# kssteven418/Q-ASR

Hardware: AMD Instinct MI355X
Metric: RTFx (audio-sec/wall-sec) QuartzNet15x5 int8 bs32 (higher is better)
Workload: dtype int8 (s8 x s8 -> i32 on MFMA; float64 fixed-point requant)

## Files before the change

### profiles/microbench/mel_cut.py

```python
import ctypes as C
import os
import subprocess
import sys
import tempfile

import numpy as np
import torch

ROOT = os.path.dirname(os.path.dirname(os.path.dirname(os.path.abspath(__file__))))
SRC = os.path.join(ROOT, 'q-asr_amd', 'csrc')
masks = [int(a) for a in sys.argv[1:]] or [0, 1, 2, 4, 8, 15, 31]
B, S, NM = 32, 80000, 64
dev = torch.device('cuda:0')
g = torch.Generator().manual_seed(0)
audio = (torch.randn(B, S, generator=g) * 0.1).to(dev)
lens = torch.full((B,), S, dtype=torch.int32, device=dev)
fb = torch.zeros(NM, 257)
edges = np.linspace(1, 256, NM + 2)
for m in range(NM):
    lo, c, hi = edges[m] ** 1.0, edges[m + 1], edges[m + 2]
    for k in range(257):
        if lo < k < hi:
            fb[m, k] = (k - lo) / (c - lo) if k <= c else (hi - k) / (hi - c)
fb = fb.to(dev)
win = torch.hann_window(320, periodic=False).to(dev)
tmp = tempfile.mkdtemp()
for mask in masks:
    so = os.path.join(tmp, f'fe{mask}.so')
    subprocess.check_call(['/opt/rocm/bin/hipcc', '--offload-arch=gfx950', '-O3', '-std=c++17', '-shared', '-fPIC',
                           f'-DMEL_CUT={mask}', '-I', os.path.join(ROOT, 'include'), '-o', so,
                           os.path.join(SRC, 'qasr_frontend.hip')])
    lib = C.CDLL(so)
    lib.qasr_frontend_frames.restype = C.c_int
    lib.qasr_frontend_workspace_bytes.restype = C.c_size_t
    T = lib.qasr_frontend_frames(S, 16)
    wsb = lib.qasr_frontend_workspace_bytes(B, S, NM)
    feats = torch.empty(B, NM, T, device=dev)
    fl = torch.empty(B, dtype=torch.int32, device=dev)
    ws = torch.empty(wsb, dtype=torch.uint8, device=dev)
    st = torch.cuda.current_stream()

    rc = lib.qasr_frontend_plan(C.c_void_p(st.cuda_stream), C.c_void_p(fb.data_ptr()), NM, C.c_void_p(ws.data_ptr()), C.c_size_t(wsb))
    assert rc == 0, rc

    def run():
        rc = lib.qasr_frontend_mel_planned(C.c_void_p(st.cuda_stream), C.c_void_p(audio.data_ptr()), C.c_void_p(lens.data_ptr()), B, S,
# ... 15 lines not shown
```

### q-asr_amd/csrc/qasr_decoder.hip

```cpp
#include "qasr_sep2_impl.h"

namespace qasr {

struct DecP {
  const int8_t* x;
  const int8_t* w;
  const int32_t* bias;
  const float* sb;
  const int32_t* lens;
  int32_t* lens_out;
  int32_t* acc_dbg;
  float* logits;
  float* logp;
  int32_t* tokens;
  float* frame_score;
  int cin, cin_pad, x_unsigned, B, T, Tp, ncls;
};

#define DEC_NT 512
#define DEC_TT 32

__global__ void __launch_bounds__(DEC_NT) k_dec(DecP p) {
  extern __shared__ __attribute__((aligned(16))) unsigned char smem[];
  const int tid = threadIdx.x, lane = tid & 63, h = lane >> 5;
  const int wave = __builtin_amdgcn_readfirstlane(tid >> 6);
  const int b = blockIdx.x, t0 = blockIdx.y * DEC_TT;
  lds_u8* const Xd = (lds_u8*)smem;
  int* const red = (int*)(smem + (size_t)p.cin_pad * 32);
  float* const lg = (float*)(red + 8 * 32 * 33);
  if (blockIdx.y == 0 && tid == 0 && p.lens_out) p.lens_out[b] = p.lens[b];
  const unsigned flip = p.x_unsigned ? 0x80808080u : 0u;
  for (int base = tid; base < 2 * p.cin_pad; base += 4 * DEC_NT) {
    v4i r[4];
#pragma unroll
    for (int u = 0; u < 4; ++u) {
      const int g = min(base + u * DEC_NT, 2 * p.cin_pad - 1), c = min(g >> 1, p.cin - 1), half = g & 1;
      r[u] = *(const v4i*)(p.x + ((size_t)b * p.cin + c) * p.Tp + t0 + 16 * half);
    }
#pragma unroll
    for (int u = 0; u < 4; ++u) {
      const int g = base + u * DEC_NT;
      if (g < 2 * p.cin_pad) {
        const int c = g >> 1, half = g & 1;
        v4i v = r[u];
        v[0] ^= flip, v[1] ^= flip, v[2] ^= flip, v[3] ^= flip;
        if (c >= p.cin) v = (v4i){0, 0, 0, 0};
        *(lds_v4i*)(Xd + c * 32 + 16 * half) = v;
      }
    }
  }
  __syncthreads();
  const int nks = p.cin_pad >> 5, per = nks >> 3;
  const lds_u8* const xd_lane = Xd + sep2_a_lane_off(lane);
  v16i acc;
#pragma unroll
  for (int r = 0; r < 16; ++r) acc[r] = 0;
  for (int i = 0; i < per; ++i) {
    const int ks = wave * per + i;
    const v4i a = sep2_a_frag(xd_lane, ks);
    const v4i wf = *w_frag(p.w, p.cin_pad, 0, ks);
    acc = __builtin_amdgcn_mfma_i32_32x32x32_i8(a, wf, acc, 0, 0, 0);
  }
#pragma unroll
  for (int r = 0; r < 16; ++r) red[(wave * 32 + mfma32_row(r, h)) * 33 + (lane & 31)] = acc[r];
  __syncthreads();
#pragma unroll
  for (int pass = 0; pass < 2; ++pass) {
    const int f = 16 * pass + (tid >> 5), c = tid & 31;
    int a = p.bias[c];
#pragma unroll
    for (int w = 0; w < 8; ++w) a += red[(w * 32 + f) * 33 + c];
    const int t = t0 + f;
    if (c < p.ncls && t < p.T) {
      if (p.acc_dbg) p.acc_dbg[((size_t)b * p.ncls + c) * p.Tp + t] = a;
      const float z = mul_f32_unfused((float)a, p.sb[c]);
      lg[f * 33 + c] = z;
      if (p.logits) p.logits[((size_t)b * p.T + t) * p.ncls + c] = z;
    }
  }
  __syncthreads();
  if (tid < DEC_TT && t0 + tid < p.T) {
    const float* x = lg + tid * 33;
    float m = x[0];
    int am = 0;
    for (int c = 1; c < p.ncls; ++c) {
      const float v = x[c];
      if (v > m) { m = v; am = c; }
    }
    float s = 0.f;
    for (int c = 0; c < p.ncls; ++c) s += expf(x[c] - m);
    const float ls = logf(s);
    const size_t row = (size_t)b * p.T + t0 + tid;
    if (p.logp)
      for (int c = 0; c < p.ncls; ++c) p.logp[row * p.ncls + c] = (x[c] - m) - ls;
    if (p.tokens) p.tokens[row] = am;
    if (p.frame_score) p.frame_score[row] = 0.0f - ls;
  }
}

bool decoder_fusable(const SepP& p) {
  return p.K == 0 && p.dense_k <= 1 && p.n_panes == 0 && (p.e.flags & QASR_F_LOGITS) && p.e.cout <= 32 && p.cin_pad % 256 == 0 &&
         p.cin_pad <= 2048 && p.e.Tp % DEC_TT == 0;
}

int launch_decoder(hipStream_t s, const SepP& q, float* logp, int32_t* tokens, int32_t* lens_out, bool keep_logits,
                   float* frame_score) {
  if (!decoder_fusable(q) || !q.x || !q.w || !q.bias || !q.e.sb || !q.e.lens || q.e.B < 1 || q.e.T > q.e.Tp) return QASR_ERR_ARG;
  DecP p{};
  p.x = q.x, p.w = q.w, p.bias = q.bias, p.sb = q.e.sb, p.lens = q.e.lens, p.lens_out = lens_out;
  p.acc_dbg = q.e.acc_dbg;
  p.logits = keep_logits ? q.e.logits : nullptr;
  p.logp = logp, p.tokens = tokens, p.frame_score = frame_score;
  p.cin = q.cin, p.cin_pad = q.cin_pad, p.x_unsigned = q.pw_unsigned;
  p.B = q.e.B, p.T = q.e.T, p.Tp = q.e.Tp, p.ncls = q.e.cout;
  const size_t smem = (size_t)p.cin_pad * 32 + sizeof(int) * 8 * 32 * 33 + sizeof(float) * 32 * 33;
  static int attr_dev = -1;
  int dev = 0;
  (void)hipGetDevice(&dev);
  if (attr_dev != dev) {
    (void)hipFuncSetAttribute((const void*)k_dec, hipFuncAttributeMaxDynamicSharedMemorySize, 160 * 1024);
    attr_dev = dev;
  }
  hipLaunchKernelGGL(k_dec, dim3(p.B, p.Tp / DEC_TT), dim3(DEC_NT), smem, s, p);
  return QASR_OK;
}

}
```

### q-asr_amd/csrc/qasr_engine.hip

```cpp
#include <algorithm>
#include <cstdarg>
#include <cstdio>
#include <cstdlib>
#include <cstring>
#include <string>
#include <type_traits>
#include <vector>

#include "qasr_internal.h"

#include <unordered_map>

using namespace qasr;

__global__ void __launch_bounds__(256) k_unpack6(const uint8_t* __restrict__ in, int8_t* __restrict__ out, size_t n_quads) {
  for (size_t q = blockIdx.x * (size_t)blockDim.x + threadIdx.x; q < n_quads; q += (size_t)gridDim.x * blockDim.x) {
    const unsigned w = in[3 * q] | ((unsigned)in[3 * q + 1] << 8) | ((unsigned)in[3 * q + 2] << 16);
    unsigned o = 0;
#pragma unroll
    for (int i = 0; i < 4; ++i) {
      const int c = (int)((w >> (6 * i)) & 0x3f);
      o |= (unsigned)(((c ^ 0x20) - 0x20) & 0xff) << (8 * i);
    }
    ((unsigned*)out)[q] = o;
// ... 56 lines not shown
  std::vector<std::vector<int32_t*>> acc_dbg;
  std::vector<hipEvent_t> ev;
  bool timed = false;
  bool fuse = true;
  std::vector<int> fused_dw;
  std::vector<char> skip;
  bool fuse_stem = true;
  bool stem = false;
  bool fuse_norm = true;
  double* norm_stats = nullptr;
  size_t norm_stats_bytes = 0;
  int norm_tiles = 0, norm_frames = 0;
  int fe_launches = 0;
  const int32_t* cur_lens = nullptr;
  bool fuse_dec = true;
  std::vector<char> rq_skip;
  std::vector<char> dec_skip;
  std::vector<char> dec_wide;
  void* decw_ws = nullptr;
  size_t decw_ws_bytes = 0;
  bool tile128 = true;
  int res_tile = 128;
  bool dense_tile128 = true;
  bool wide_tiles = false;
  int mask_skip = -1;
  int sep_gen = 2;
  bool forwarded = false;
  bool use_graph = false;
  hipGraphExec_t gexec = nullptr;
  const void* gkey[8] = {nullptr, nullptr, nullptr, nullptr, nullptr, nullptr, nullptr, nullptr};
// ... 95 lines not shown
  for (uint32_t d = 0; d < h.n_domains; ++d)
    if (e->domT[d] <= 0) return fail(QASR_ERR_ARG, "input of %d frames is too short for domain %u", T0, d);
  e->tens.resize(h.n_tensors);
  for (uint32_t i = 0; i < h.n_tensors; ++i) {
    TensorRT& t = e->tens[i];
    t.d = e->tdesc[i];
    t.T = e->domT[t.d.domain];
    t.Tp = rup(t.T, 64);
    t.bytes = (t.d.dtype == QASR_DT_F32) ? (size_t)B * t.T * t.d.channels * 4 : (size_t)B * t.d.channels * t.Tp * dt_size(t.d.dtype);
    t.bytes = (t.bytes + 255) / 256 * 256;
  }
  e->fused_dw.assign(h.n_ops, -1);
  e->skip.assign(h.n_ops, 0);
  e->dec_skip.assign(h.n_ops, 0);
  e->dec_wide.assign(h.n_ops, 0);
  e->rq_skip.assign(h.n_ops, 0);
  if (e->fuse)
    for (uint32_t oi = 0; oi + 1 < h.n_ops; ++oi) {
      const qasr_op_desc& d = e->ops[oi];
      const qasr_op_desc& q = e->ops[oi + 1];
      if (d.kind != QASR_OP_DW || q.kind != QASR_OP_PW) continue;
      const uint32_t same_pad = d.dilation > 1 ? (d.dilation * d.kernel) / 2 - 1 : d.kernel / 2;
      if (d.stride != 1 || d.padding != same_pad || !(d.kernel & 1) || !sep_supported((int)d.kernel, (int)d.dilation)) continue;
      if (d.outs[1].tensor >= 0 || d.outs[0].mode != 1 || q.in != d.outs[0].tensor) continue;
      if (e->tdesc[d.outs[0].tensor].last_use != (int)oi + 1 || (d.flags & QASR_F_EXACT_Z)) continue;
      e->fused_dw[oi + 1] = (int)oi;
      e->skip[oi] = 1;
    }
  e->B = B;
  e->T0 = T0;
// ... 161 lines not shown
  return QASR_OK;
}
int qasr_debug_timeline(void* dev_buf, size_t capacity_work_groups) {
  if (dev_buf && (capacity_work_groups < 1 || capacity_work_groups > (1u << 22))) return fail(QASR_ERR_ARG, "debug_timeline: capacity");
  qasr::g_prof = (long long*)dev_buf;
  qasr::g_prof_mode = dev_buf ? 1 : 0;
  qasr::g_prof_cap = dev_buf ? (int)capacity_work_groups : 0;
  return QASR_OK;
}

void qasr_engine_default_opts(qasr_engine_opts* o) {
  if (!o) return;
  memset(o, 0, sizeof *o);
  o->struct_size = (uint32_t)sizeof *o;
  o->fuse_dw = o->fuse_stem = o->fuse_decoder = o->res_tile128 = o->dense_tile128 = o->fuse_norm = o->mask_skip = -1;
}

#define QASR_SIDE_BY_SIDE_QUEUES 8
#define QASR_RES_TILE_FEW_CHAINS 64
static int res_tile_default() {
  long q = 4;
  if (const char* g = getenv("GPU_MAX_HW_QUEUES")) {
    char* end = nullptr;
    const long v = strtol(g, &end, 10);
    if (end != g && v >= 1) q = v;
  }
  return q >= QASR_SIDE_BY_SIDE_QUEUES ? 128 : QASR_RES_TILE_FEW_CHAINS;
}

int qasr_engine_create(const void* blob, size_t n, int device, int debug, qasr_engine** out) {
// ... 26 lines not shown
    char why[256];
    if (qasr_blob_check(blob, n, why, sizeof why) != QASR_OK) return fail(QASR_ERR_BLOB, "%s", why);
  }
  qasr_blob_header h;
  memcpy(&h, blob, sizeof h);
  HIPCHK(hipSetDevice(device));
  qasr_engine* e = new qasr_engine();
  e->device = device;
  e->debug = (debug & 1) != 0;
  e->timing = (debug & 3) != 0;
  auto tri = [](int32_t v, bool dflt) { return v < 0 ? dflt : v != 0; };
  e->fuse = tri(o.fuse_dw, true);
  e->fuse_stem = tri(o.fuse_stem, true);
  e->fuse_dec = tri(o.fuse_decoder, true);
  e->fuse_norm = tri(o.fuse_norm, true);
  e->wide_tiles = o.tile_frames >= 64;
  e->tile128 = o.tile_frames == 128;
  e->res_tile = o.res_tile128 < 0 ? res_tile_default() : (o.res_tile128 ? 128 : 64);
  e->dense_tile128 = tri(o.dense_tile128, true);
  e->sep_gen = o.sep_gen == 1 ? 1 : 2;
  e->mask_skip = o.mask_skip < 0 ? -1 : (o.mask_skip != 0);
  e->use_graph = o.graph > 0;
  if (getenv("QASR_NO_FUSE")) e->fuse = false;
  if (getenv("QASR_WIDE_TILES")) { e->wide_tiles = true; e->tile128 = true; }
  if (const char* g = getenv("QASR_TILE128")) e->tile128 = atoi(g) != 0;
  if (const char* g = getenv("QASR_RES_TILE128")) e->res_tile = atoi(g) != 0 ? 128 : 64;
  if (const char* g = getenv("QASR_RES_TILE")) {
    const int v = atoi(g);
    if (v == 32 || v == 64 || v == 128) e->res_tile = v;
  }
// ... 72 lines not shown
    if (bk.gexec) (void)hipGraphExecDestroy(bk.gexec);
  for (void* p : e->rs.owned) dev_free(e, p);
  free_plan(e);
  for (auto v : e->ev) (void)hipEventDestroy(v);
  dev_free(e, e->dblob);
  dev_free(e, e->dexp);
  delete e;
}

int qasr_engine_num_ops(const qasr_engine* e) { return e ? (int)e->h.n_ops : -1; }

int qasr_engine_num_launches(const qasr_engine* e) {
  if (!e || !e->B || !e->forwarded) return -1;
  int n = (e->stem ? 0 : 1) + e->fe_launches;
  for (uint32_t oi = 0; oi < e->h.n_ops; ++oi) {
    if (e->skip[oi] || e->dec_skip[oi] || e->rq_skip[oi] || (e->stem && oi >= 1 && oi <= 2)) continue;
    n += e->dec_wide[oi] ? 2 : 1;
  }
  return n + (e->ctc_on ? 1 : 0);
}

int qasr_engine_out_frames(const qasr_engine* e, int T) {
  if (!e) return -1;
  std::vector<int> dT(e->h.n_domains);
  dT[0] = T;
  for (uint32_t d = 1; d < e->h.n_domains; ++d) dT[d] = conv_out_len(dT[e->doms[d].parent], e->doms[d]);
  const qasr_op_desc& last = e->ops[e->h.n_ops - 1];
  return dT[e->tdesc[last.in].domain];
}

static void build_sep(qasr_engine* e, uint32_t oi, SepP& p) {
// ... 107 lines not shown
  QuantInP qi{};
  DwP dw{};
  SepP pw{};
  build_quant_in(e, 0, qi);
  build_dw(e, 1, dw);
  build_sep(e, 2, pw);
  int rc = launch_stem(s, qi, dw, pw, (const qasr_domain_desc*)(e->dblob + e->h.domains_off), (int)e->h.n_domains, e->cur_lens,
                       e->lens_all, e->norm_tiles ? e->norm_stats : nullptr, e->norm_tiles, e->norm_frames);
  return rc ? fail(rc, "k_stem launch") : QASR_OK;
}

static int launch_op(qasr_engine* e, hipStream_t s, uint32_t oi, float* logp, int32_t* tokens, int32_t* lens_out) {
  const qasr_op_desc& op = e->ops[oi];
  const int B = e->B;
  if (e->skip[oi]) return QASR_OK;
  if (e->stem && oi <= 2) return oi == 0 ? stem_launch(e, s) : QASR_OK;
  const TensorRT& tin = e->tens[op.in];
  switch (op.kind) {
    case QASR_OP_QUANT_IN: {
      QuantInP p{};
      build_quant_in(e, oi, p);
      launch_quant_in(s, p);
      break;
    }
    case QASR_OP_DW: {
      DwP p{};
      build_dw(e, oi, p);
      launch_dw(s, p);
      break;
    }
// ... 2 lines not shown
      build_sep(e, oi, p);
      if (e->fuse_dec && (op.flags & QASR_F_LOGITS) && oi + 1 < e->h.n_ops && e->ops[oi + 1].kind == QASR_OP_LOGSOFTMAX &&
          e->ops[oi + 1].in == op.outs[0].tensor && decoder_fusable(p)) {
        int rc = launch_decoder(s, p, logp, tokens, lens_out, e->debug, e->ctc_fs);
        if (rc) return fail(rc, "op %u: decoder launch", oi);
        e->dec_skip[oi + 1] = 1;
        break;
      }
      if (e->fuse_dec && (op.flags & QASR_F_LOGITS) && oi + 1 < e->h.n_ops && e->ops[oi + 1].kind == QASR_OP_LOGSOFTMAX &&
          e->ops[oi + 1].in == op.outs[0].tensor && decoder_wide_fusable(p)) {
        int rc = launch_decoder_wide(s, p, logp, tokens, lens_out, e->debug, e->decw_ws, e->decw_ws_bytes, e->ctc_fs);
        if (rc) return fail(rc, "op %u: wide decoder launch", oi);
        e->dec_skip[oi + 1] = 1;
        e->dec_wide[oi] = 1;
        break;
      }
      int rc = launch_sep(s, p);
      if (rc) return fail(rc, "op %u: no k_sep instantiation for K=%d dilation=%d (or bad launch shape)", oi, p.K, p.dilation);
      break;
    }
    case QASR_OP_DENSE: {
      if (op.flags & QASR_F_TAPMAJOR) {
        SepP p{};
        build_sep(e, oi, p);
        int rc = launch_sep(s, p);
        if (rc) return fail(rc, "op %u: dense conv has no k_sep launch shape", oi);
        break;
      }
      DenseP p{};
      p.x = (const int8_t*)tin.ptr;
// ... 1023 lines not shown
    HIPCHK(hipEventSynchronize(b));
    float ms = 0.f;
    HIPCHK(hipEventElapsedTime(&ms, a, b));
    ms_per_launch[oi] = ms / reps;
  }
  (void)hipEventDestroy(a);
  (void)hipEventDestroy(b);
  return QASR_OK;
}

int qasr_engine_op_label(qasr_engine* e, int op, char* buf, size_t cap) {
  if (!e || !buf || cap < 8 || op < 0 || op >= (int)e->h.n_ops) return fail(QASR_ERR_ARG, "op_label: bad argument");
  const qasr_op_desc& d = e->ops[op];
  const char* name = "?";
  if (e->skip[op]) name = "(fused into the next op)";
  else if (e->dec_skip[op]) name = "(fused into the previous op)";
  else if (e->rq_skip[op]) name = "(served by the previous k_requant launch)";
  else if (e->stem && op <= 2) name = op == 0 ? "k_stem" : "(fused into the first op)";
  else switch (d.kind) {
    case QASR_OP_QUANT_IN: name = "k_quant_in"; break;
    case QASR_OP_DW: name = "k_dw"; break;
    case QASR_OP_DENSE:
      if (d.flags & QASR_F_TAPMAJOR) {
        SepP p{};
        build_sep(e, (uint32_t)op, p);
        sep_kernel_label(p, buf, cap);
        return QASR_OK;
      }
      name = "k_dense";
      break;
    case QASR_OP_LOGSOFTMAX: name = "k_logsoftmax"; break;
// ... 271 lines not shown
```

### q-asr_amd/csrc/qasr_internal.h

```cpp
#pragma once
#include <hip/hip_runtime.h>
#include <stdint.h>

#include "../../include/qasr.h"

namespace qasr {

struct OutP {
  void* ptr;
  const double* mtab;
  double m;
  int lo, hi, mode;
  int pad_;
};

struct PaneP {
  const int8_t* x;
  const int8_t* w;
  const int32_t* bias;
  const double* m;
  const float* sb;
  int32_t* acc_dbg;
  int cin, cin_pad, x_unsigned, pad_;
};
// ... 97 lines not shown
size_t frontend_stats_bytes(int B, int S, int n_mels);
struct RaggedFront {
  int pitch, T_pad;
  const int32_t* shp;
};
int frontend_mel_stats(hipStream_t s, const float* audio, const int32_t* audio_lens, int B, int S, const float* fb,
                       const float* window, int n_mels, float preemph, int pad_to, float* feats, int32_t* feat_lens,
                       const void* workspace, size_t workspace_bytes, double* stats, int* n_tiles, int* n_frames,
                       const RaggedFront* rg = nullptr);
int frontend_mel_planned_ragged(hipStream_t s, const float* audio, const int32_t* audio_lens, int B, int S, const float* fb,
                                const float* window, int n_mels, float preemph, int pad_to, float* feats, int32_t* feat_lens,
                                const void* workspace, size_t workspace_bytes, const RaggedFront& rg);
bool decoder_fusable(const SepP& p);
int launch_decoder(hipStream_t s, const SepP& p, float* logp, int32_t* tokens, int32_t* lens_out, bool keep_logits,
                   float* frame_score = nullptr);
#define QASR_DECW_MAX_CLASSES 8192
bool decoder_wide_fusable(const SepP& p);
size_t decoder_wide_ws_bytes(int B, int Tp);
int launch_decoder_wide(hipStream_t s, const SepP& p, float* logp, int32_t* tokens, int32_t* lens_out, bool keep_logits,
                        void* ws, size_t ws_bytes, float* frame_score = nullptr);
int launch_ctc(hipStream_t s, const int32_t* tokens, const float* frame_score, const int32_t* lens, int B, int T, int blank,
               const qasr_ctc_out& out, const int32_t* t_act = nullptr);
int launch_topn(hipStream_t s, const qasr_ctc_topn_args& a);
size_t beam_workspace_bytes(int B, int T, int W);
int launch_beam(hipStream_t s, const qasr_ctc_beam_args& a);
int launch_beam_lm(hipStream_t s, const qasr_ctc_beam_lm_args& a);
int launch_beam_boost(hipStream_t s, const qasr_ctc_beam_boost_args& a);
size_t align_workspace_bytes(int P, int T, int max_labels);
int launch_align(hipStream_t s, const qasr_ctc_align_args& a);
size_t align_band_workspace_bytes(int P, int T, int band_states);
// ... 32 lines not shown
```

### q-asr_amd/csrc/qasr_sep2_impl.h

```cpp
#pragma once
#include <algorithm>
#include <cstdio>
#include <cstdlib>
#include <type_traits>

#include "qasr_device.h"

namespace qasr {

typedef int v2i __attribute__((ext_vector_type(2)));
typedef unsigned char __attribute__((address_space(3))) lds_u8;
typedef unsigned __attribute__((address_space(3))) lds_u32;
typedef v2i __attribute__((address_space(3))) lds_v2i;
typedef v4i __attribute__((address_space(3))) lds_v4i;

#define SEP2_NT 512
#ifndef SEP2_WPE
#define SEP2_WPE 2
#endif
#define SEP2_CH 128

template <int K, int TT>
struct Sep2Geo {
  static constexpr int PAD = K / 2;
// ... 154 lines not shown
      } else {
        if (r1) sep2_load_wg(&wf[4 * g], r1 + 256 * g);
      }
    }
    __builtin_amdgcn_sched_barrier(0);
  });
}

struct Sep2PassP {
  int bias, pbias;
  double Mo[QASR_MAX_OUTS];
  double Mm, Mp;
  float sbm, sbp;
};

template <int K, int NG, int NGP, int NP, bool DBG, int TT, int DIL = 1, bool SKIP = false>
__device__ __forceinline__ void sep2_body(const SepP& p, const int b, const int t0, const bool stamp_wg, const int wg_id) {
  using G = Sep2Geo<K, TT / DIL>;
  constexpr bool RES = NGP > 0;
  static_assert(DIL == 1 || (DIL == 2 && !RES && TT >= 64), "dilation 2: plain layers, 64- / 128-frame tiles");
  constexpr int MT = TT / 32;
  constexpr int NU = G::NU, S = G::S, NS = G::NS;
  constexpr int CIN_PAD = 128 * NG, PCIN_PAD = 128 * NGP;
  constexpr int RCH = 16 / DIL, GCH = SEP2_CH / DIL;
  constexpr int NCHUNK = (CIN_PAD + GCH - 1) / GCH;
  constexpr int NPGR = DIL == 1 ? G::NPG : (TT + 2 * DIL * G::HALO) / 16;
  constexpr int NPT = (RCH * NPGR + 63) / 64, NTG = RCH * G::KS / 16, NTT = (NTG + 63) / 64;
  static_assert(DIL == 1 || (8 * NPGR == G::WLEN && (RCH * G::KS) % 16 == 0), "dilation 2: window / tap granules");
  extern __shared__ __attribute__((aligned(16))) unsigned char smem[];
  const EpiP& e = p.e;
  int tid_ = threadIdx.x;
  asm volatile("" : "+v"(tid_));
  const int tid = tid_, lane = tid & 63, h = lane >> 5;
  const int wave = __builtin_amdgcn_readfirstlane(tid >> 6);
// ... 420 lines not shown
          }
        }
      };
      auto unit_values = [&](v16i* a, int ps, int mt0, auto v0c, auto v1c) __attribute__((always_inline)) {
        constexpr int v0 = decltype(v0c)::value, v1 = decltype(v1c)::value;
        sep2_for<v0, v1>([&](auto vc) {
          constexpr int v = decltype(vc)::value, mt = v / 16, r = v % 16;
          q4[r & 3] = rq_clamp(a[mt][r], pps[ps].Mo[0], olo, ohi);
          if constexpr ((r & 3) == 3) P[r >> 2] = pack4b(q4[0], q4[1], q4[2], q4[3]);
          if constexpr (r == 15) {
            const auto s02 = __builtin_amdgcn_permlane32_swap(P[0], P[2], false, false);
            const auto s13 = __builtin_amdgcn_permlane32_swap(P[1], P[3], false, false);
            v4i pk = {(int)s02[0], (int)s02[1], (int)s13[0], (int)s13[1]};
            if (t0 + 32 * (mt0 + mt + 1) > lim) pk = sep2_mask16(pk, lim - (t0 + 32 * (mt0 + mt) + 16 * h));
            *(v4i*)(optr + ((size_t)b * ecout + 256 * ps + co_l) * eTp + t0 + 32 * (mt0 + mt) + 16 * h) = pk;
          }
        });
      };
      auto u_ps = [](int u) constexpr { return u < NUN0 ? u / NH : NP - 1; };
      auto u_mh = [](int u) constexpr { return (SPLIT && u >= NUN0 - 1) ? 1 : MH; };
      auto u_mt0 = [](int u) constexpr { return u < NUN0 ? (u % NH) * MH : (NH - 1) * MH + 1; };
      sep2_for<0, NUN>([&](auto uc) {
        constexpr int u = decltype(uc)::value, ps = u_ps(u), mh = u_mh(u), mt0 = u_mt0(u);
        constexpr int AB = mh >= 2 ? 1 : 2, NSL = 4 * NG * mh;
        v16i* const cur = accs[u & 1];
#pragma unroll
        for (int mt = 0; mt < mh; ++mt)
#pragma unroll
          for (int r = 0; r < 16; ++r) cur[mt][r] = pps[ps].bias;
        const v4i* const wnext = (u < NUN0 && u % NH == NH - 1 && ps + 1 < NP) ? w_frag(p.w, CIN_PAD, 256 * (ps + 1) + co_l, 0) : nullptr;
        if constexpr (u > 0) unit_finish(accs[(u - 1) & 1], u_ps(u - 1), u_mt0(u - 1), std::integral_constant<int, u_mh(u - 1)>{});
        sep2_gemm_cb<mh, NG, 0, AB>(cur, wf, xd_lane + mt0 * (CIN_PAD * 32), CIN_PAD * 32, nullptr, wnext, [&](auto qc) {
          if constexpr (u > 0) {
            constexpr int NV = 16 * u_mh(u - 1), VPS = (NV + NSL - 1) / NSL;
            constexpr int q = decltype(qc)::value, v0 = q * VPS < NV ? q * VPS : NV, v1 = (q + 1) * VPS < NV ? (q + 1) * VPS : NV;
            unit_values(accs[(u - 1) & 1], u_ps(u - 1), u_mt0(u - 1), std::integral_constant<int, v0>{}, std::integral_constant<int, v1>{});
          }
        });
        STAMP2();
      });
      unit_finish(accs[(NUN - 1) & 1], NP - 1, u_mt0(NUN - 1), std::integral_constant<int, u_mh(NUN - 1)>{});
      unit_values(accs[(NUN - 1) & 1], NP - 1, u_mt0(NUN - 1), std::integral_constant<int, 0>{}, std::integral_constant<int, 16 * u_mh(NUN - 1)>{});
      STAMP2();
    }
  }
  if constexpr (!PIPED) {
#pragma unroll
  for (int ps = 0; ps < NP; ++ps) {
    const int cbase = 256 * ps;
    const int co = cbase + co_l, cor = co;
    constexpr bool co_ok = true;
    const bool more = ps + 1 < NP;
    const v4i* const wnext = more ? w_frag(p.w, CIN_PAD, co + 256, 0) : nullptr;
    const v4i* const wpane = RES ? w_frag(p.panes[0].w, PCIN_PAD, cor, 0) : nullptr;
    const Sep2PassP& pp = pps[ps];
    v16i acc[MT];
#pragma unroll
    for (int mt = 0; mt < MT; ++mt)
#pragma unroll
      for (int r = 0; r < 16; ++r) acc[mt][r] = pp.bias;
// ... 189 lines not shown
```

### q-asr_amd/qasr/engine.py

```python
import ctypes as C
import os

import numpy as np
import torch

HERE = os.path.dirname(os.path.abspath(__file__))
LIB_PATH = os.environ.get('QASR_LIB', os.path.join(HERE, 'libqasr_hip.so'))

SYMBOLS = ['qasr_blob_check', 'qasr_engine_create', 'qasr_engine_create_ex', 'qasr_engine_default_opts', 'qasr_engine_destroy', 'qasr_engine_forward', 'qasr_engine_forward_audio', 'qasr_engine_out_frames',
           'qasr_engine_num_ops', 'qasr_engine_num_launches', 'qasr_engine_read_acc', 'qasr_engine_read_tensor', 'qasr_engine_last_op_ms',
           'qasr_engine_time_ops', 'qasr_engine_run_op', 'qasr_engine_op_label',
           'qasr_frontend_mel', 'qasr_frontend_plan', 'qasr_frontend_mel_planned', 'qasr_frontend_frames',
           'qasr_frontend_workspace_bytes', 'qasr_pw_conv_acc',
           'qasr_dw_conv_acc', 'qasr_dense_conv_acc', 'qasr_requant', 'qasr_dyn_range', 'qasr_dyn_range_percentile', 'qasr_dyn_residue_codes', 'qasr_dyn_act_params', 'qasr_dyn_requant',
           'qasr_dyn_quant_in', 'qasr_dyn_conv_params', 'qasr_sep_layer', 'qasr_quantile2', 'qasr_quantile_workspace_bytes', 'qasr_debug_prof',
           'qasr_debug_timeline', 'qasr_ctc_collapse', 'qasr_engine_attach_ctc', 'qasr_ctc_topn', 'qasr_ctc_beam_workspace_bytes', 'qasr_ctc_beam',
           'qasr_lm_check', 'qasr_ctc_beam_lm', 'qasr_boost_check', 'qasr_ctc_beam_boost', 'qasr_ctc_align_workspace_bytes', 'qasr_ctc_align',
           'qasr_ctc_align_band_workspace_bytes', 'qasr_ctc_align_band',
           'qasr_engine_reserve', 'qasr_engine_forward_ragged', 'qasr_engine_forward_ragged_audio', 'qasr_engine_ragged_stats',
           'qasr_ragged_bucket_frames', 'qasr_ragged_envelope_frames',
           'qasr_resample_check', 'qasr_resample', 'qasr_resample_out_samples', 'qasr_longform_cut', 'qasr_longform_stitch',
           'qasr_stream_state_bytes', 'qasr_stream_push', 'qasr_stream_window', 'qasr_stream_emit',
           'qasr_last_error', 'qasr_version']

# ... 938 lines not shown
    for n in ('labels', 'start', 'nframes', 'score', 'n_new_labels', 'status', 'total_frames', 'utt_score'):
        setattr(a, n, getattr(out, n).data_ptr())
    if out.tail_labels is not None:
        assert out.tail_labels.dtype == torch.int32 and out.tail_labels.is_contiguous() and out.tail_labels.shape[0] == B, 'stream_emit: out'
        _i32dev(out.tail_n, B, 'stream_emit: out')
        a.Ptail, a.tail_labels, a.tail_n = out.tail_labels.shape[1], out.tail_labels.data_ptr(), out.tail_n.data_ptr()
    with torch.cuda.device(dev):
        _check(lib.qasr_stream_emit(_stream_ptr(stream), C.byref(a)), 'qasr_stream_emit')
    return out


class Engine:

    def __init__(self, blob: bytes, device=0, debug=False, timing=False, wide_tiles=False,
                 graph=False, tile=None, sep_gen=None, fuse_dw=None, fuse_stem=None, fuse_decoder=None, res_tile128=None,
                 dense_tile128=None, fuse_norm=None, legacy_create=False, mask_skip=None):
        lib = load_library()
        if not torch.cuda.is_available():
            raise QasrError('no GPU: the integer engine needs an MI355X (there is no CPU fallback)')
        self.lib = lib
        self.device = torch.device('cuda', device)
        self._blob = blob
        self._h = C.c_void_p()
        buf = (C.c_char * len(blob)).from_buffer_copy(blob)
        o = EngineOpts()
        lib.qasr_engine_default_opts(C.byref(o))
        assert o.struct_size == C.sizeof(EngineOpts), 'qasr_engine_opts: header and binding disagree'
        o.debug = int(bool(debug)) | (2 if timing else 0)
        o.tile_frames = int(tile) if tile else (128 if wide_tiles else 32)
        o.sep_gen = int(sep_gen or 0)
        for name, v in (('fuse_dw', fuse_dw), ('fuse_stem', fuse_stem), ('fuse_decoder', fuse_decoder),
                        ('res_tile128', res_tile128), ('dense_tile128', dense_tile128), ('fuse_norm', fuse_norm),
                        ('mask_skip', mask_skip)):
            if v is not None:
                setattr(o, name, int(bool(v)))
        o.graph = int(bool(graph))
        self.opts = o
        if legacy_create:
            bits = o.debug | (8 if o.tile_frames == 128 else 0) | (16 if graph else 0)
            _check(lib.qasr_engine_create(C.cast(buf, C.c_void_p), len(blob), device, bits, C.byref(self._h)), 'qasr_engine_create')
        else:
            _check(lib.qasr_engine_create_ex(C.cast(buf, C.c_void_p), len(blob), device, C.byref(o), C.byref(self._h)),
                   'qasr_engine_create_ex')
        self.debug = debug
        self.n_ops = lib.qasr_engine_num_ops(self._h)
        hdr = np.frombuffer(blob[:40], dtype=np.uint32)
        self.feat_in, self.n_classes = int(hdr[4]), int(hdr[5])
        self.B = self.T = None
        self._ctc = None
        self._ctc_auto = False
# ... 421 lines not shown
```

Measured before the change: 292,100.

## Fuse CTC decoder pointwise and log-softmax into the last encoder 1x1 layer

Adds a k_sep2_dec kernel in which the final 512->1024 pointwise encoder layer writes its int8 output tile into LDS through a tail hook. The same workgroup then runs the decoder 1x1 MFMA over that tile, the bias/scale reduction and the log-softmax/argmax. This removes the separate k_dec launch and the global re-read of the 1024-channel activation. In exchange the tile grows to a large LDS footprint (about 160 KB), which may lower occupancy of the encoder layer, and the extra decoder work lengthens each workgroup.

New measurement: 293,100, median of 4. About the same (+0.3%).

```diff
diff --git a/profiles/chain_ends.py b/profiles/chain_ends.py
--- /dev/null
+++ b/profiles/chain_ends.py
@@ -0,0 +1,125 @@
+#!/usr/bin/env python3
+import argparse
+import csv
+import glob
+import hashlib
+import json
+import os
+import shutil
+import statistics
+import subprocess
+import sys
+import tempfile
+
+ROOT = os.path.dirname(os.path.dirname(os.path.abspath(__file__)))
+ENDS = ('qasr::k_mel<', 'qasr::k_stem(', 'qasr::k_sep2<0, 4, 0, 4, false, 64, 1>', 'qasr::k_sep2_dec(', 'qasr::k_dec(',
+        'qasr::k_sep2<75, 4, 0, 2, false, 128, 1>')
+
+
+def lib_path(name):
+    return os.path.join(ROOT, 'q-asr_amd', 'qasr', f'libqasr_{name}.so')
+
+
+def bench_cmd(steps, warmup, extra=()):
+    return [sys.executable, os.path.join(ROOT, 'bench.py'), '--gpus', '1', '--steps', str(steps), '--warmup', str(warmup), *extra]
+
+
+def run_bench(build, queues, steps, warmup, extra=(), prefix=()):
+    env = dict(os.environ, QASR_LIB=lib_path(build), GPU_MAX_HW_QUEUES=str(queues))
+    p = subprocess.run([*prefix, *bench_cmd(steps, warmup, extra)], capture_output=True, text=True, env=env, timeout=400)
+    if p.returncode:
+        print(f'{build} (queues {queues}): FAILED rc={p.returncode}\n{p.stderr[-2000:]}', flush=True)
+        return None
+    d = json.loads([l for l in p.stdout.strip().splitlines() if l.startswith('{')][-1])
+    streams = [l.split('] ', 1)[1] for l in p.stderr.splitlines() if 'streams finished at' in l]
+    return dict(ms_per_step=d['ms_per_step'], rtfx=d['value'], streams=streams[0] if streams else None)
+
+
+def sha(path):
+    return hashlib.sha256(open(path, 'rb').read()).hexdigest()
+
+
+def main():
+    ap = argparse.ArgumentParser()
+    ap.add_argument('out')
+    ap.add_argument('--parent', default='parent')
+    ap.add_argument('--this', default='hip')
+    ap.add_argument('--rounds', type=int, default=3)
+    ap.add_argument('--steps', type=int, default=50)
+    ap.add_argument('--warmup', type=int, default=5)
+    ap.add_argument('--queues', type=int, nargs='+', default=[4, 8])
+    ap.add_argument('--stats', action='store_true')
+    a = ap.parse_args()
+    res = json.load(open(a.out)) if os.path.exists(a.out) else {}
+    builds = (a.parent, a.this)
+
+    def save():
+        with open(a.out, 'w') as fh:
+            json.dump(res, fh, indent=1)
+
+    if a.stats:
+        q = a.queues[0]
+        res['kernel_stats'] = dict(GPU_MAX_HW_QUEUES=q, steps=a.steps, warmup=a.warmup, rows={})
+        for build in builds:
+            tmp = tempfile.mkdtemp()
+            r = run_bench(build, q, a.steps, a.warmup, prefix=('rocprofv3', '--kernel-trace', '--stats', '--output-format', 'csv', '-d', tmp, '-o', 'p', '--'))
+            if r is None:
+                return 1
+            files = glob.glob(os.path.join(tmp, '**', '*kernel_stats.csv'), recursive=True)
+            rows = list(csv.reader(open(files[0])))
+            keep = [rows[0]] + [x for x in rows[1:] if 'qasr::' in x[0]]
+            with open(os.path.splitext(a.out)[0] + f'_kernel_stats_{build}.csv', 'w', newline='') as fh:
+                csv.writer(fh).writerows(keep)
+            ends = {}
+            for x in keep[1:]:
+                if any(k in x[0] for k in ENDS):
+                    name = x[0].replace('void ', '').split('(')[0]
+                    ends[name] = dict(calls=int(x[1]), mean_us=float(x[3]) / 1e3, min_us=float(x[5]) / 1e3, max_us=float(x[6]) / 1e3,
+                                      sigma_us=float(x[7]) / 1e3)
+            res['kernel_stats']['rows'][build] = dict(ms_per_step_under_rocprof=r['ms_per_step'], ends=ends)
+            shutil.rmtree(tmp, ignore_errors=True)
+            for k, v in ends.items():
+                print(f"{build:8s} {k:50s} {v['calls']:5d} calls  mean {v['mean_us']:7.2f}  max {v['max_us']:7.2f}  sigma {v['sigma_us']:6.2f} us", flush=True)
+            save()
+        return 0
+
+    runs = res.setdefault('runs', [])
+    for q in a.queues:
+        for r in range(a.rounds):
+            for build in builds:
+                rec = run_bench(build, q, a.steps, a.warmup)
+                if rec is None:
+                    return 1
+                rec.update(build=build, round=r, GPU_MAX_HW_QUEUES=q, steps=a.steps, warmup=a.warmup)
+                runs.append(rec)
+                print(f"{build:8s} queues {q:2d} round {r}  {rec['ms_per_step']:.4f} ms/step  {rec['streams']}", flush=True)
+                save()
+    summary = res.setdefault('summary', {})
+    for q in a.queues:
+        per = {b: sorted(x['ms_per_step'] for x in runs if x['build'] == b and x['GPU_MAX_HW_QUEUES'] == q) for b in builds}
+        summary[str(q)] = {b: dict(min=v[0], median=statistics.median(v), max=v[-1]) for b, v in per.items() if v}
+    if all(b in summary.get(str(a.queues[0]), {}) for b in builds):
+        s = summary[str(a.queues[0])]
+        summary['faster_than_every_parent_run'] = s[a.this]['max'] < s[a.parent]['min']
+    save()
+    hashes = res.setdefault('output_sha256', {})
+    for build in builds:
+        hashes[build] = {}
+        for extra in ((), ('--gather', 'logits')):
+            tmp = tempfile.mkdtemp()
+            if run_bench(build, a.queues[0], min(a.steps, 10), 2, extra=(*extra, '--dump-outputs', tmp)) is None:
+                return 1
+            for f in sorted(glob.glob(os.path.join(tmp, '*.npy'))):
+                name = os.path.basename(f)
+                if extra or name != 'log_probs.npy':
+                    h = sha(f)
+                    assert hashes[build].setdefault(name, h) == h, f'{build}: {name} differs between the two runs'
+            shutil.rmtree(tmp, ignore_errors=True)
+    res['outputs_identical'] = hashes[a.parent] == hashes[a.this] and len(hashes[a.this]) >= 3
+    save()
+    print(json.dumps(dict(summary=summary, outputs_identical=res['outputs_identical'], files=sorted(hashes[a.this])), indent=1), flush=True)
+    return 0 if res['outputs_identical'] else 2
+
+
+if __name__ == '__main__':
+    sys.exit(main())
diff --git a/profiles/microbench/mel_cut.py b/profiles/microbench/mel_cut.py
--- a/profiles/microbench/mel_cut.py
+++ b/profiles/microbench/mel_cut.py
@@ -27,9 +27,13 @@
 tmp = tempfile.mkdtemp()
 for mask in masks:
     so = os.path.join(tmp, f'fe{mask}.so')
-    subprocess.check_call(['/opt/rocm/bin/hipcc', '--offload-arch=gfx950', '-O3', '-std=c++17', '-shared', '-fPIC',
-                           f'-DMEL_CUT={mask}', '-I', os.path.join(ROOT, 'include'), '-o', so,
-                           os.path.join(SRC, 'qasr_frontend.hip')])
+    pre = os.path.join(os.environ.get('MEL_CUT_LIBS', tmp), f'fe{mask}.so')
+    if os.path.exists(pre):
+        so = pre
+    else:
+        subprocess.check_call(['/opt/rocm/bin/hipcc', '--offload-arch=gfx950', '-O3', '-std=c++17', '-shared', '-fPIC',
+                               f'-DMEL_CUT={mask}', '-I', os.path.join(ROOT, 'include'), '-o', so,
+                               os.path.join(SRC, 'qasr_frontend.hip')])
     lib = C.CDLL(so)
     lib.qasr_frontend_frames.restype = C.c_int
     lib.qasr_frontend_workspace_bytes.restype = C.c_size_t
diff --git a/q-asr_amd/csrc/qasr_decoder.hip b/q-asr_amd/csrc/qasr_decoder.hip
--- a/q-asr_amd/csrc/qasr_decoder.hip
+++ b/q-asr_amd/csrc/qasr_decoder.hip
@@ -20,9 +20,65 @@
 #define DEC_NT 512
 #define DEC_TT 32
 
+template <int NTL>
+__device__ __forceinline__ void dec_partial(const DecP& p, const lds_u8* Xd, int stride, int lane, int wave, v16i (&acc)[NTL]) {
+  const int nks = p.cin_pad >> 5, per = nks >> 3;
+  const lds_u8* const xd_lane = Xd + sep2_a_lane_off(lane);
+#pragma unroll
+  for (int n = 0; n < NTL; ++n)
+#pragma unroll
+    for (int r = 0; r < 16; ++r) acc[n][r] = 0;
+  for (int i = 0; i < per; ++i) {
+    const int ks = wave * per + i;
+    const v4i wf = *w_frag(p.w, p.cin_pad, 0, ks);
+#pragma unroll
+    for (int n = 0; n < NTL; ++n) {
+      const v4i a = sep2_a_frag(xd_lane + n * stride, ks);
+      acc[n] = __builtin_amdgcn_mfma_i32_32x32x32_i8(a, wf, acc[n], 0, 0, 0);
+    }
+  }
+}
+__device__ __forceinline__ void dec_put_partial(int* red, const v16i& acc, int lane, int wave) {
+  const int h = lane >> 5;
+#pragma unroll
+  for (int r = 0; r < 16; ++r) red[(wave * 32 + mfma32_row(r, h)) * 33 + (lane & 31)] = acc[r];
+}
+__device__ __forceinline__ void dec_reduce(const DecP& p, const int* red, float* lg, int b, int t0, int tid) {
+#pragma unroll
+  for (int pass = 0; pass < 2; ++pass) {
+    const int f = 16 * pass + (tid >> 5), c = tid & 31;
+    int a = p.bias[c];
+#pragma unroll
+    for (int w = 0; w < 8; ++w) a += red[(w * 32 + f) * 33 + c];
+    const int t = t0 + f;
+    if (c < p.ncls && t < p.T) {
+      if (p.acc_dbg) p.acc_dbg[((size_t)b * p.ncls + c) * p.Tp + t] = a;
+      const float z = mul_f32_unfused((float)a, p.sb[c]);
+      lg[f * 33 + c] = z;
+      if (p.logits) p.logits[((size_t)b * p.T + t) * p.ncls + c] = z;
+    }
+  }
+}
+__device__ __forceinline__ void dec_softmax(const DecP& p, const float* x, int b, int t) {
+  float m = x[0];
+  int am = 0;
+  for (int c = 1; c < p.ncls; ++c) {
+    const float v = x[c];
+    if (v > m) { m = v; am = c; }
+  }
+  float s = 0.f;
+  for (int c = 0; c < p.ncls; ++c) s += expf(x[c] - m);
+  const float ls = logf(s);
+  const size_t row = (size_t)b * p.T + t;
+  if (p.logp)
+    for (int c = 0; c < p.ncls; ++c) p.logp[row * p.ncls + c] = (x[c] - m) - ls;
+  if (p.tokens) p.tokens[row] = am;
+  if (p.frame_score) p.frame_score[row] = 0.0f - ls;
+}
+
 __global__ void __launch_bounds__(DEC_NT) k_dec(DecP p) {
   extern __shared__ __attribute__((aligned(16))) unsigned char smem[];
-  const int tid = threadIdx.x, lane = tid & 63, h = lane >> 5;
+  const int tid = threadIdx.x, lane = tid & 63;
   const int wave = __builtin_amdgcn_readfirstlane(tid >> 6);
   const int b = blockIdx.x, t0 = blockIdx.y * DEC_TT;
   lds_u8* const Xd = (lds_u8*)smem;
@@ -50,52 +106,60 @@
     }
   }
   __syncthreads();
-  const int nks = p.cin_pad >> 5, per = nks >> 3;
-  const lds_u8* const xd_lane = Xd + sep2_a_lane_off(lane);
-  v16i acc;
-#pragma unroll
-  for (int r = 0; r < 16; ++r) acc[r] = 0;
-  for (int i = 0; i < per; ++i) {
-    const int ks = wave * per + i;
-    const v4i a = sep2_a_frag(xd_lane, ks);
-    const v4i wf = *w_frag(p.w, p.cin_pad, 0, ks);
-    acc = __builtin_amdgcn_mfma_i32_32x32x32_i8(a, wf, acc, 0, 0, 0);
-  }
-#pragma unroll
-  for (int r = 0; r < 16; ++r) red[(wave * 32 + mfma32_row(r, h)) * 33 + (lane & 31)] = acc[r];
+  v16i acc[1];
+  dec_partial<1>(p, Xd, 0, lane, wave, acc);
+  dec_put_partial(red, acc[0], lane, wave);
   __syncthreads();
-#pragma unroll
-  for (int pass = 0; pass < 2; ++pass) {
-    const int f = 16 * pass + (tid >> 5), c = tid & 31;
-    int a = p.bias[c];
-#pragma unroll
-    for (int w = 0; w < 8; ++w) a += red[(w * 32 + f) * 33 + c];
-    const int t = t0 + f;
-    if (c < p.ncls && t < p.T) {
-      if (p.acc_dbg) p.acc_dbg[((size_t)b * p.ncls + c) * p.Tp + t] = a;
-      const float z = mul_f32_unfused((float)a, p.sb[c]);
-      lg[f * 33 + c] = z;
-      if (p.logits) p.logits[((size_t)b * p.T + t) * p.ncls + c] = z;
-    }
-  }
+  dec_reduce(p, red, lg, b, t0, tid);
   __syncthreads();
-  if (tid < DEC_TT && t0 + tid < p.T) {
-    const float* x = lg + tid * 33;
-    float m = x[0];
-    int am = 0;
-    for (int c = 1; c < p.ncls; ++c) {
-      const float v = x[c];
-      if (v > m) { m = v; am = c; }
-    }
-    float s = 0.f;
-    for (int c = 0; c < p.ncls; ++c) s += expf(x[c] - m);
-    const float ls = logf(s);
-    const size_t row = (size_t)b * p.T + t0 + tid;
-    if (p.logp)
-      for (int c = 0; c < p.ncls; ++c) p.logp[row * p.ncls + c] = (x[c] - m) - ls;
-    if (p.tokens) p.tokens[row] = am;
-    if (p.frame_score) p.frame_score[row] = 0.0f - ls;
-  }
+  if (tid < DEC_TT && t0 + tid < p.T) dec_softmax(p, lg + tid * 33, b, t0 + tid);
+}
+
+#define TAIL_TT 64
+#define TAIL_CIN 512
+#define TAIL_CMID 1024
+#define TAIL_IMG (TAIL_TT * TAIL_CIN)
+#define TAIL_RED (TAIL_IMG + TAIL_TT * TAIL_CMID)
+#define TAIL_LG (TAIL_RED + 4 * 8 * 32 * 33)
+#define TAIL_SMEM (TAIL_LG + 4 * TAIL_TT * 33)
+static_assert(TAIL_SMEM <= 160 * 1024, "k_sep2_dec: LDS budget");
+
+struct Sep2DecTail {
+  static constexpr bool on = true;
+  const DecP& d;
+  unsigned char* smem;
+  lds_u8* lds;
+  unsigned flip;
+  __device__ __forceinline__ void put(int mt, int ch, int h, v4i pk) const {
+    pk[0] ^= flip, pk[1] ^= flip, pk[2] ^= flip, pk[3] ^= flip;
+    *(lds_v4i*)(lds + TAIL_IMG + mt * (32 * TAIL_CMID) + ch * 32 + 16 * h) = pk;
+  }
+  __device__ __forceinline__ void run(int b, int t0, int tid) const {
+    const int lane = tid & 63, wave = __builtin_amdgcn_readfirstlane(tid >> 6);
+    int* const red = (int*)(smem + TAIL_RED);
+    float* const lg = (float*)(smem + TAIL_LG);
+    if (t0 == 0 && tid == 0 && d.lens_out) d.lens_out[b] = d.lens[b];
+    __syncthreads();
+    v16i acc[2];
+    dec_partial<2>(d, lds + TAIL_IMG, 32 * TAIL_CMID, lane, wave, acc);
+#pragma unroll
+    for (int n = 0; n < 2; ++n) {
+      if (n) __syncthreads();
+      dec_put_partial(red, acc[n], lane, wave);
+      __syncthreads();
+      dec_reduce(d, red, lg + n * (DEC_TT * 33), b, t0 + DEC_TT * n, tid);
+    }
+    __syncthreads();
+    if (tid < TAIL_TT && t0 + tid < d.T) dec_softmax(d, lg + tid * 33, b, t0 + tid);
+  }
+};
+
+__global__ void __launch_bounds__(SEP2_NT, SEP2_WPE) k_sep2_dec(SepP p, DecP d) {
+  extern __shared__ __attribute__((aligned(16))) unsigned char smem[];
+  static_assert(SEP2_NT == DEC_NT, "the decoder's thread layout");
+  const Sep2DecTail tail{d, smem, (lds_u8*)smem, d.x_unsigned ? 0x80808080u : 0u};
+  sep2_body<0, TAIL_CIN / 128, 0, TAIL_CMID / 256, false, TAIL_TT, 1, false, Sep2DecTail>(
+      p, blockIdx.x, blockIdx.y * TAIL_TT, blockIdx.x == 0 && blockIdx.y == 1, blockIdx.y * gridDim.x + blockIdx.x, tail);
 }
 
 bool decoder_fusable(const SepP& p) {
@@ -103,16 +167,20 @@
          p.cin_pad <= 2048 && p.e.Tp % DEC_TT == 0;
 }
 
-int launch_decoder(hipStream_t s, const SepP& q, float* logp, int32_t* tokens, int32_t* lens_out, bool keep_logits,
-                   float* frame_score) {
-  if (!decoder_fusable(q) || !q.x || !q.w || !q.bias || !q.e.sb || !q.e.lens || q.e.B < 1 || q.e.T > q.e.Tp) return QASR_ERR_ARG;
-  DecP p{};
+static void dec_params(DecP& p, const SepP& q, float* logp, int32_t* tokens, int32_t* lens_out, bool keep_logits, float* frame_score) {
   p.x = q.x, p.w = q.w, p.bias = q.bias, p.sb = q.e.sb, p.lens = q.e.lens, p.lens_out = lens_out;
   p.acc_dbg = q.e.acc_dbg;
   p.logits = keep_logits ? q.e.logits : nullptr;
   p.logp = logp, p.tokens = tokens, p.frame_score = frame_score;
   p.cin = q.cin, p.cin_pad = q.cin_pad, p.x_unsigned = q.pw_unsigned;
   p.B = q.e.B, p.T = q.e.T, p.Tp = q.e.Tp, p.ncls = q.e.cout;
+}
+
+int launch_decoder(hipStream_t s, const SepP& q, float* logp, int32_t* tokens, int32_t* lens_out, bool keep_logits,
+                   float* frame_score) {
+  if (!decoder_fusable(q) || !q.x || !q.w || !q.bias || !q.e.sb || !q.e.lens || q.e.B < 1 || q.e.T > q.e.Tp) return QASR_ERR_ARG;
+  DecP p{};
+  dec_params(p, q, logp, tokens, lens_out, keep_logits, frame_score);
   const size_t smem = (size_t)p.cin_pad * 32 + sizeof(int) * 8 * 32 * 33 + sizeof(float) * 32 * 33;
   static int attr_dev = -1;
   int dev = 0;
@@ -125,4 +193,33 @@
   return QASR_OK;
 }
 
-}
+bool decoder_tail_fusable(const SepP& enc, const SepP& dec) {
+  const EpiP& e = enc.e;
+  if (!decoder_fusable(dec) || dec.e.acc_dbg || dec.cin != TAIL_CMID || dec.cin_pad != TAIL_CMID) return false;
+  if (enc.gen != 2 || !sep2_shape_ok(enc) || enc.K != 0 || enc.cin_pad != TAIL_CIN || e.cout != TAIL_CMID || enc.tile < 64) return false;
+  if (enc.mask_skip || e.acc_dbg || enc.dw_acc_dbg || g_prof) return false;
+  return e.n_outs == 1 && e.outs[0].ptr == (const void*)dec.x && e.B == dec.e.B && e.T == dec.e.T && e.Tp == dec.e.Tp && e.Tp % TAIL_TT == 0;
+}
+
+int launch_decoder_tail(hipStream_t s, const SepP& enc, const SepP& dec, float* logp, int32_t* tokens, int32_t* lens_out, float* frame_score) {
+  if (!decoder_tail_fusable(enc, dec) || !enc.x || !enc.w || !dec.x || !dec.w || !dec.bias || !dec.e.sb || !dec.e.lens || dec.e.B < 1 ||
+      dec.e.T > dec.e.Tp)
+    return QASR_ERR_ARG;
+  DecP d{};
+  dec_params(d, dec, logp, tokens, lens_out, false, frame_score);
+  SepP q = enc;
+  q.prof = nullptr;
+  q.prof_mode = 0;
+  q.prof_cap = 0;
+  static int attr_dev = -1;
+  int dev = 0;
+  (void)hipGetDevice(&dev);
+  if (attr_dev != dev) {
+    (void)hipFuncSetAttribute((const void*)k_sep2_dec, hipFuncAttributeMaxDynamicSharedMemorySize, 160 * 1024);
+    attr_dev = dev;
+  }
+  hipLaunchKernelGGL(k_sep2_dec, dim3(q.e.B, q.e.Tp / TAIL_TT, 1), dim3(SEP2_NT), (size_t)TAIL_SMEM, s, q, d);
+  return QASR_OK;
+}
+
+}
diff --git a/q-asr_amd/csrc/qasr_engine.hip b/q-asr_amd/csrc/qasr_engine.hip
--- a/q-asr_amd/csrc/qasr_engine.hip
+++ b/q-asr_amd/csrc/qasr_engine.hip
@@ -94,6 +94,8 @@
   int fe_launches = 0;
   const int32_t* cur_lens = nullptr;
   bool fuse_dec = true;
+  bool fuse_tail = true;
+  std::vector<char> tail_skip;
   std::vector<char> rq_skip;
   std::vector<char> dec_skip;
   std::vector<char> dec_wide;
@@ -219,6 +221,7 @@
   e->skip.assign(h.n_ops, 0);
   e->dec_skip.assign(h.n_ops, 0);
   e->dec_wide.assign(h.n_ops, 0);
+  e->tail_skip.assign(h.n_ops, 0);
   e->rq_skip.assign(h.n_ops, 0);
   if (e->fuse)
     for (uint32_t oi = 0; oi + 1 < h.n_ops; ++oi) {
@@ -410,6 +413,7 @@
   memset(o, 0, sizeof *o);
   o->struct_size = (uint32_t)sizeof *o;
   o->fuse_dw = o->fuse_stem = o->fuse_decoder = o->res_tile128 = o->dense_tile128 = o->fuse_norm = o->mask_skip = -1;
+  o->reserved[0] = -1;
 }
 
 #define QASR_SIDE_BY_SIDE_QUEUES 8
@@ -466,6 +470,7 @@
   e->fuse_stem = tri(o.fuse_stem, true);
   e->fuse_dec = tri(o.fuse_decoder, true);
   e->fuse_norm = tri(o.fuse_norm, true);
+  e->fuse_tail = tri(o.reserved[0], true);
   e->wide_tiles = o.tile_frames >= 64;
   e->tile128 = o.tile_frames == 128;
   e->res_tile = o.res_tile128 < 0 ? res_tile_default() : (o.res_tile128 ? 128 : 64);
@@ -568,7 +573,7 @@
   if (!e || !e->B || !e->forwarded) return -1;
   int n = (e->stem ? 0 : 1) + e->fe_launches;
   for (uint32_t oi = 0; oi < e->h.n_ops; ++oi) {
-    if (e->skip[oi] || e->dec_skip[oi] || e->rq_skip[oi] || (e->stem && oi >= 1 && oi <= 2)) continue;
+    if (e->skip[oi] || e->dec_skip[oi] || e->tail_skip[oi] || e->rq_skip[oi] || (e->stem && oi >= 1 && oi <= 2)) continue;
     n += e->dec_wide[oi] ? 2 : 1;
   }
   return n + (e->ctc_on ? 1 : 0);
@@ -706,6 +711,7 @@
   const qasr_op_desc& op = e->ops[oi];
   const int B = e->B;
   if (e->skip[oi]) return QASR_OK;
+  if (e->tail_skip[oi]) return QASR_OK;
   if (e->stem && oi <= 2) return oi == 0 ? stem_launch(e, s) : QASR_OK;
   const TensorRT& tin = e->tens[op.in];
   switch (op.kind) {
@@ -738,6 +744,21 @@
         e->dec_skip[oi + 1] = 1;
         e->dec_wide[oi] = 1;
         break;
+      }
+      if (e->fuse_dec && e->fuse_tail && !e->debug && !e->timing && !e->rs.on && oi + 2 < e->h.n_ops) {
+        const qasr_op_desc &d1 = e->ops[oi + 1], &d2 = e->ops[oi + 2];
+        if (d1.kind == QASR_OP_PW && (d1.flags & QASR_F_LOGITS) && d1.in == op.outs[0].tensor && d2.kind == QASR_OP_LOGSOFTMAX &&
+            d2.in == d1.outs[0].tensor) {
+          SepP pd{};
+          build_sep(e, oi + 1, pd);
+          if (decoder_tail_fusable(p, pd)) {
+            int rc = launch_decoder_tail(s, p, pd, logp, tokens, lens_out, e->ctc_fs);
+            if (rc) return fail(rc, "op %u: decoder launch inside the previous layer's", oi + 1);
+            e->tail_skip[oi + 1] = 1;
+            e->dec_skip[oi + 2] = 1;
+            break;
+          }
+        }
       }
       int rc = launch_sep(s, p);
       if (rc) return fail(rc, "op %u: no k_sep instantiation for K=%d dilation=%d (or bad launch shape)", oi, p.K, p.dilation);
@@ -1791,7 +1812,7 @@
   const qasr_op_desc& d = e->ops[op];
   const char* name = "?";
   if (e->skip[op]) name = "(fused into the next op)";
-  else if (e->dec_skip[op]) name = "(fused into the previous op)";
+  else if (e->dec_skip[op] || e->tail_skip[op]) name = "(fused into the previous op)";
   else if (e->rq_skip[op]) name = "(served by the previous k_requant launch)";
   else if (e->stem && op <= 2) name = op == 0 ? "k_stem" : "(fused into the first op)";
   else switch (d.kind) {
diff --git a/q-asr_amd/csrc/qasr_internal.h b/q-asr_amd/csrc/qasr_internal.h
--- a/q-asr_amd/csrc/qasr_internal.h
+++ b/q-asr_amd/csrc/qasr_internal.h
@@ -135,6 +135,9 @@
 bool decoder_fusable(const SepP& p);
 int launch_decoder(hipStream_t s, const SepP& p, float* logp, int32_t* tokens, int32_t* lens_out, bool keep_logits,
                    float* frame_score = nullptr);
+bool decoder_tail_fusable(const SepP& enc, const SepP& dec);
+int launch_decoder_tail(hipStream_t s, const SepP& enc, const SepP& dec, float* logp, int32_t* tokens, int32_t* lens_out,
+                        float* frame_score = nullptr);
 #define QASR_DECW_MAX_CLASSES 8192
 bool decoder_wide_fusable(const SepP& p);
 size_t decoder_wide_ws_bytes(int B, int Tp);
diff --git a/q-asr_amd/csrc/qasr_sep2_impl.h b/q-asr_amd/csrc/qasr_sep2_impl.h
--- a/q-asr_amd/csrc/qasr_sep2_impl.h
+++ b/q-asr_amd/csrc/qasr_sep2_impl.h
@@ -192,10 +192,15 @@
   float sbm, sbp;
 };
 
-template <int K, int NG, int NGP, int NP, bool DBG, int TT, int DIL = 1, bool SKIP = false>
-__device__ __forceinline__ void sep2_body(const SepP& p, const int b, const int t0, const bool stamp_wg, const int wg_id) {
+struct Sep2NoTail {
+  static constexpr bool on = false;
+};
+template <int K, int NG, int NGP, int NP, bool DBG, int TT, int DIL = 1, bool SKIP = false, class TAIL = Sep2NoTail>
+__device__ __forceinline__ void sep2_body(const SepP& p, const int b, const int t0, const bool stamp_wg, const int wg_id,
+                                          const TAIL tail = TAIL{}) {
   using G = Sep2Geo<K, TT / DIL>;
   constexpr bool RES = NGP > 0;
+  static_assert(!TAIL::on || (K == 0 && !RES && !DBG && !SKIP && TT == 64), "the tail hook: the bare 1x1 form on 64-frame tiles");
   static_assert(DIL == 1 || (DIL == 2 && !RES && TT >= 64), "dilation 2: plain layers, 64- / 128-frame tiles");
   constexpr int MT = TT / 32;
   constexpr int NU = G::NU, S = G::S, NS = G::NS;
@@ -646,6 +651,7 @@
             v4i pk = {(int)s02[0], (int)s02[1], (int)s13[0], (int)s13[1]};
             if (t0 + 32 * (mt0 + mt + 1) > lim) pk = sep2_mask16(pk, lim - (t0 + 32 * (mt0 + mt) + 16 * h));
             *(v4i*)(optr + ((size_t)b * ecout + 256 * ps + co_l) * eTp + t0 + 32 * (mt0 + mt) + 16 * h) = pk;
+            if constexpr (TAIL::on) tail.put(mt0 + mt, 256 * ps + co_l, h, pk);
           }
         });
       };
@@ -676,6 +682,8 @@
       STAMP2();
     }
   }
+  static_assert(!TAIL::on || PIPED, "the tail hook sits in the pipelined epilogue");
+  if constexpr (TAIL::on) tail.run(b, t0, tid);
   if constexpr (!PIPED) {
 #pragma unroll
   for (int ps = 0; ps < NP; ++ps) {
diff --git a/q-asr_amd/qasr/engine.py b/q-asr_amd/qasr/engine.py
--- a/q-asr_amd/qasr/engine.py
+++ b/q-asr_amd/qasr/engine.py
@@ -976,7 +976,7 @@
 
     def __init__(self, blob: bytes, device=0, debug=False, timing=False, wide_tiles=False,
                  graph=False, tile=None, sep_gen=None, fuse_dw=None, fuse_stem=None, fuse_decoder=None, res_tile128=None,
-                 dense_tile128=None, fuse_norm=None, legacy_create=False, mask_skip=None):
+                 dense_tile128=None, fuse_norm=None, legacy_create=False, mask_skip=None, fuse_tail=None):
         lib = load_library()
         if not torch.cuda.is_available():
             raise QasrError('no GPU: the integer engine needs an MI355X (there is no CPU fallback)')
@@ -996,6 +996,8 @@
                         ('mask_skip', mask_skip)):
             if v is not None:
                 setattr(o, name, int(bool(v)))
+        if fuse_tail is not None:
+            o.reserved[0] = int(bool(fuse_tail))
         o.graph = int(bool(graph))
         self.opts = o
         if legacy_create:
```
